# borglab/gtsam

Hardware: NVIDIA H100
Metric: LM iterations/sec (linearize+solve) on BAL-style graph (higher is better)
Workload: dtype f32 Jacobians + f64 solve

## Files before the change

gtsam_b200/csrc/engine.cu:

```cuda
#include <algorithm>
#include <chrono>
#include <climits>
#include <cmath>
#include <cstdlib>
#include <dlfcn.h>
#include <cstring>
#include <limits>
#include <memory>
#include <thread>

#include "kernels.cuh"

namespace b200 {

static thread_local std::string g_err;

template <class F>
static void parallel_chunks(int64_t n, F f) {
  int nt = (int)std::min<int64_t>(std::max(1u, std::thread::hardware_concurrency()), 16);
  if (const char* e = getenv("B200_SETUP_THREADS")) nt = std::min(16, std::max(1, atoi(e)));
  nt = (int)std::min<int64_t>(nt, std::max<int64_t>(1, n / 65536));
  if (nt <= 1) { f((int64_t)0, n, 0); return; }
  std::vector<std::thread> pool;
  for (int t = 0; t < nt; t++) pool.emplace_back([=, &f]() { f(n * t / nt, n * (t + 1) / nt, t); });
// ... 163 lines not shown
  for (auto& g : p->groups) {
    if (!g.count) continue;
    PhaseScope ps(p, g.count >= 4096 ? PH_LINEARIZE : PH_LINEARIZE_MINOR);
    const int nb = (int)((g.count + 127) / 128);
    const bool proj = g.type == B200_FACTOR_PROJECTION_CAL3S2 || g.type == B200_FACTOR_SFM_BUNDLER;
    if (proj && p->lin_variant == 4) {
      if (g.type == B200_FACTOR_PROJECTION_CAL3S2)
        DISPATCH_JT(p, launch_k(linearize_kernel<B200_FACTOR_PROJECTION_CAL3S2, JT, 4>, dim3(nb), dim3(128), 0, st, view(g), ectx(p, p->d_values)));
      else
        DISPATCH_JT(p, launch_k(linearize_kernel<B200_FACTOR_SFM_BUNDLER, JT, 4>, dim3(nb), dim3(128), 0, st, view(g), ectx(p, p->d_values)));
    } else
    DISPATCH_JT(p, DISPATCH_TYPE(g.type, (launch_k(linearize_kernel<TY, JT>, dim3(nb), dim3(128), 0, st, view(g), ectx(p, p->d_values)))));
    p->ctx->launches++;
  }
  B200_CUDA(cudaGetLastError());
  p->linearized = true;
  p->hdiag_valid = false;
  return B200_OK;
}

static int enqueue_hdiag(b200_problem* p) {
  cudaStream_t st = p->ctx->stream;
  B200_CUDA(cudaMemsetAsync(p->d_hdiag, 0, (size_t)p->ndelta * sizeof(double), st));
  for (auto& g : p->groups) {
    if (!g.count) continue;
    const int nb = (int)((g.count + 127) / 128);
    if (g.type == B200_FACTOR_JACOBIAN) launch_k(hdiag_jacobian_kernel, dim3(nb), dim3(128), 0, st, jview(g), (const int*)p->d_var_dof, p->d_hdiag);
    else if (g.type == B200_FACTOR_HESSIAN) launch_k(hdiag_hessian_kernel, dim3(nb), dim3(128), 0, st, jview(g), (const int*)p->d_var_dof, p->d_hdiag);
    else DISPATCH_JT(p, DISPATCH_TYPE(g.type, (launch_k(hdiag_kernel<TY, JT>, dim3(nb), dim3(128), 0, st, view(g), p->d_var_dof, p->d_hdiag))));
    p->ctx->launches++;
  }
  B200_CUDA(cudaGetLastError());
  return allreduce_sum(p, p->d_hdiag, (size_t)p->ndelta);
}

static int enqueue_solve(b200_problem* p, bool damped, int diagonal, double min_diag, double max_diag) {
  cudaStream_t st = p->ctx->stream;
  b200_ctx* ctx = p->ctx;
  const TreeView t = tview(p);
  {
    PhaseScope ps(p, PH_MEMSET);
    if (p->zero_doubles) B200_CUDA(cudaMemsetAsync(p->d_arena, 0, (size_t)p->zero_doubles * sizeof(double), st));
    if (p->df_sync_ints) B200_CUDA(cudaMemsetAsync(p->d_df_sync, 0, (size_t)p->df_sync_ints * sizeof(int), st));
    if (p->topx_doubles && p->d_topx) B200_CUDA(cudaMemsetAsync(p->d_topx, 0, (size_t)p->topx_doubles * sizeof(double), st));
  }
  {
    PhaseScope ps(p, PH_ASSEMBLE);
    for (auto& g : p->groups) {
      if (!g.n_nonleaf) continue;
      const int nb = (int)((g.count + 127) / 128);
      if (g.type == B200_FACTOR_JACOBIAN) launch_k(assemble_jacobian_kernel, dim3(nb), dim3(128), 0, st, jview(g), t);
      else if (g.type == B200_FACTOR_HESSIAN) launch_k(assemble_hessian_kernel, dim3(nb), dim3(128), 0, st, jview(g), t);
      else DISPATCH_JT(p, DISPATCH_TYPE(g.type, (launch_k(assemble_kernel<TY, JT>, dim3(nb), dim3(128), 0, st, view(g), t))));
      ctx->launches++;
    }
  }
  if (damped) {
    PhaseScope ps(p, PH_DAMP);
    if (diagonal && !p->hdiag_valid) { const int rc = enqueue_hdiag(p); if (rc) return rc; p->hdiag_valid = true; }
    launch_k(damp_kernel, dim3((int)((p->ndelta + 255) / 256)), dim3(256), 0, st, p->d_arena, p->d_diag_index, (int)p->ndelta, p->d_lambda,
                                                                diagonal ? p->d_hdiag.get() : nullptr, min_diag, max_diag);
    ctx->launches++;
  }
  if (p->n_fused) {
    PhaseScope ps(p, PH_LEAF);
    GroupTable gt;
    for (size_t gi = 0; gi < p->groups.size(); gi++) gt.g[gi] = view(p->groups[gi]);
    const double* hd = (damped && diagonal) ? p->d_hdiag.get() : nullptr;
    if (p->leaf_run_end[0] > p->leaf_run_begin[0]) {
      const int nr = p->leaf_run_end[0] - p->leaf_run_begin[0], nb = (nr + kWarpsPerBlock - 1) / kWarpsPerBlock;
      const size_t sm = (size_t)kWarpsPerBlock * p->leaf_lb_cap * sizeof(double);
      DISPATCH_JT(p, launch_k(leaf_fused_kernel<JT>, dim3(nb), dim3(kWarpsPerBlock * 32), sm, st, t, gt, p->d_fused_list, p->d_fused_run_ptr + p->leaf_run_begin[0], nr,
                                                           p->d_fused_fac_ptr, p->d_fused_fac, p->d_lambda, hd, min_diag, max_diag,
                                                           p->d_scalars, p->leaf_lb_cap, 0));
      ctx->launches++;
    }
    for (int kd = 1; kd <= 2 && p->schur_mma; kd++) {
      const int nr = p->leaf_run_end[kd] - p->leaf_run_begin[kd];
      if (nr <= 0) continue;
      const int* runs = p->d_fused_run_ptr + p->leaf_run_begin[kd];
      const int dc = kd == 1 ? 6 : 9, maxw = p->leaf_max_w[kd], nt8 = (maxw + 7) / 8;
      const int mmax = std::max(1, (maxw - 1) / dc), sa = (dc < 8 ? 8 : 16) * kSmPA + kSmPadA;
      const size_t jb = p->jac_f32 ? sizeof(float) : sizeof(double);
      const size_t sm = std::max((size_t)4 * (3 + 8 * nt8) * kSmKS * sizeof(double) + (size_t)4 * (2 * mmax * sa + 2 * 6 * 32) * jb,
                                 (size_t)64 * nt8 * nt8 * sizeof(double));
      bool done = false;
#define B200_LAUNCH_FUSED(DC_, T_)                                                                                                    \
      if (!done && dc == DC_ && nt8 <= T_) {                                                                                          \
        DISPATCH_JT(p, launch_k(leaf_point_fused_mma_kernel<DC_, T_, JT>, dim3(nr), dim3(128), sm, st, t, gt, (const int*)p->d_fused_list, runs, \
                 (const double*)p->d_lambda, hd, min_diag, max_diag, p->d_scalars, (const int2*)p->d_pt_tab, (const int64_t*)p->d_pt_off)); \
        done = true;                                                                                                                  \
      }
      B200_LAUNCH_FUSED(6, 4) B200_LAUNCH_FUSED(6, 5) B200_LAUNCH_FUSED(6, 7)
      B200_LAUNCH_FUSED(9, 4) B200_LAUNCH_FUSED(9, 5) B200_LAUNCH_FUSED(9, 7) B200_LAUNCH_FUSED(9, 10)
#undef B200_LAUNCH_FUSED
      if (!done) { set_error("leaf_point_fused_mma_kernel: separator wider than the compiled tile counts"); return B200_CUDA_ERROR; }
      ctx->launches++;
    }
    for (int kd = 1; kd <= 2 && !p->schur_mma; kd++) {
      if (p->leaf_run_end[kd] <= p->leaf_run_begin[kd]) continue;
      const int i0 = p->leaf_pos_begin[kd], i1 = p->leaf_pos_end[kd];
      const int nb = (int)(((int64_t)(i1 - i0) * 8 + 127) / 128);
#define B200_LAUNCH_POINT(DC_)                                                                                                        \
      DISPATCH_JT(p, launch_k(leaf_point_factor_kernel<DC_, JT>, dim3(nb), dim3(128), 0, st, t, gt, (const int*)p->d_fused_list, i0, i1, \
               (const int*)p->d_fused_fac_ptr, (const int2*)p->d_fused_fac, (const double*)p->d_lambda, hd, min_diag, max_diag,        \
               p->d_scalars, (const int2*)p->d_pt_tab, (const int64_t*)p->d_pt_off));
      if (kd == 1) { B200_LAUNCH_POINT(6) } else { B200_LAUNCH_POINT(9) }
#undef B200_LAUNCH_POINT
      ctx->launches++;
    }
  }
  if (p->n_fused && !p->schur_mma) {
    PhaseScope ps(p, PH_LEAF_SCHUR);
    GroupTable gt;
    for (size_t gi = 0; gi < p->groups.size(); gi++) gt.g[gi] = view(p->groups[gi]);
    for (int kd = 1; kd <= 2; kd++) {
      const int nr = p->leaf_run_end[kd] - p->leaf_run_begin[kd];
      if (nr <= 0) continue;
      const int* runs = p->d_fused_run_ptr + p->leaf_run_begin[kd];
      const int ntd = (p->leaf_max_w[kd] + 2) / 3, ntiles = ntd * (ntd + 1) / 2;
      const int thr = ntiles <= 96 ? 96 : 128, tpt = (ntiles + thr - 1) / thr;
#define B200_LAUNCH_SCHUR(DC_, T_, P_)                                                                                               \
      if (kd == (DC_ == 6 ? 1 : 2) && tpt == T_ && p->schur_pb == P_)                                                                \
        DISPATCH_JT(p, launch_k(leaf_point_schur_kernel<DC_, T_, P_, JT>, dim3(nr), dim3(thr), 0, st, t, gt, (const int*)p->d_fused_list, runs, \
                 (const int*)p->d_fused_fac_ptr, (const int2*)p->d_fused_fac));
      if (tpt > (kd == 1 ? 2 : 3)) { set_error("leaf_point_schur_kernel: separator wider than the compiled tile counts"); return B200_CUDA_ERROR; }
      B200_LAUNCH_SCHUR(6, 1, 4) B200_LAUNCH_SCHUR(6, 2, 4)
      B200_LAUNCH_SCHUR(6, 1, 6) B200_LAUNCH_SCHUR(6, 2, 6)
      B200_LAUNCH_SCHUR(9, 1, 4) B200_LAUNCH_SCHUR(9, 2, 4) B200_LAUNCH_SCHUR(9, 3, 4)
      B200_LAUNCH_SCHUR(9, 1, 6) B200_LAUNCH_SCHUR(9, 2, 6) B200_LAUNCH_SCHUR(9, 3, 6)
#undef B200_LAUNCH_SCHUR
      ctx->launches++;
    }
  }
  for (size_t l = 0; l < p->levels.size(); l++) {
    if ((int)l == p->n_sub_levels && ctx->world > 1 && !p->top_staged) {
      PhaseScope ps(p, PH_ALLREDUCE);
      const int rc = allreduce_sum(p, p->d_arena, (size_t)p->top_doubles);
      if (rc) return rc;
    }
    const LevelPlan& L = p->levels[l];
    auto launch_df = [&](int slot, const int4* tasks, int ntasks, bool trace) {
      DfView v;
      v.tasks = tasks; v.ntasks = ntasks;
      v.ctrl = p->d_df_sync + 2 * slot; v.done = p->d_df_sync + p->df_ctrl_ints; v.flags = v.done + p->sym.ncliques;
      v.flag_off = p->d_df_flag_off; v.expect = p->d_df_expect;
      v.trace = trace ? p->d_df_trace.get() : nullptr;
      v.winv = p->d_winv; v.winv_off = p->d_winv_off;
      v.warm_ctas = getenv("B200_DF_NO_WARM") ? 0 : 3 * ctx->sm_count;
      if (p->df_minb == 3) launch_k(front_df_kernel<3>, dim3(ntasks), dim3(kDfThreads), (size_t)kDfSmemBytes, st, t, v, p->d_scalars);
      else launch_k(front_df_kernel<2>, dim3(ntasks), dim3(kDfThreads), (size_t)kDfSmemBytes, st, t, v, p->d_scalars);
      ctx->launches++;
    };
    for (int ph = 0; ph < 2; ph++)
      if ((int)l == p->df_level[ph] && p->df_ntasks[ph] && !(ph == 1 && p->top_staged)) {
        PhaseScope ps(p, PH_ELIM_LARGE);
        launch_df(ph, p->d_df_tasks[ph], p->df_ntasks[ph], ph == 0);
      }
    if (p->top_staged)
      for (size_t s = 0; s < p->ts_level.size(); s++)
        if (p->ts_level[s] == (int)l) {
          {
            PhaseScope ps(p, PH_ALLREDUCE);
            const int rc = reduce_top_stage(p, s);
            if (rc) return rc;
          }
          if (p->ts_task_count[s]) {
            PhaseScope ps(p, PH_ELIM_LARGE);
// ... 639 lines not shown
  int64_t ngroups = 0;
  Packed pk;
  std::vector<char> fused, is_top;
  std::vector<int> clique_owner, factor_owner, top_owner;
  std::vector<int> fused_list, run_ptr;
  std::vector<int> leaf_kind;
  std::vector<std::vector<int2>> hkeys; std::vector<std::vector<int4>> hscat;
};

static int setup_symbolic(b200_problem* p, ProblemPlan& P) {
  if (const int rc = P.d ? pack_and_symbolic(P.d, &P.pk) : pack_linear(P.ld, &P.pk)) return rc;
  const int64_t n = P.d ? P.d->nvars : P.ld->nvars;
  P.ngroups = P.d ? P.d->ngroups : P.ld->ngroups + P.ld->nhgroups;
  p->nvars = n; p->nval = P.pk.val_off[n]; p->ndelta = P.pk.var_dof[n]; p->nfactors = P.pk.total;
  if (P.d) p->var_type.assign(P.d->var_type, P.d->var_type + n);
  p->groups.resize(P.ngroups);
  for (int64_t gi = 0; gi < P.ngroups; gi++) {
    auto& g = p->groups[gi];
    const PackedGroup& q = P.pk.groups[gi];
    g.type = q.type; g.noise_kind = q.noise_kind; g.per_factor = q.per_factor; g.noise_size = q.noise_size;
    g.d = q.d; g.ncols = q.ncols; g.arity = q.arity; g.meas = q.meas; g.count = q.count; g.pos = q.pos;
    g.robust_kind = q.robust_kind; g.robust_param = q.robust_param;
    g.col0[0] = 0;
    for (int a = 0; a < B200_JACOBIAN_MAX_ARITY; a++) g.col0[a + 1] = g.col0[a] + (a < q.arity ? q.dims[a] : 0);
    g.col0[q.arity + 1] = g.col0[q.arity] + 1;
  }
  p->sym = std::move(P.pk.sym);
  return B200_OK;
}
static int setup_values(b200_problem* p, ProblemPlan& P) {
  if (P.d) {
    B200_CUDA(upload(p->d_values, P.d->values, (size_t)p->nval, p->ctx->stream));
    B200_CUDA(p->d_new_values.alloc(p->nval));
    B200_CUDA(upload(p->d_val_off, P.pk.val_off, p->ctx->stream));
    B200_CUDA(upload(p->d_var_type, p->var_type, p->ctx->stream));
    B200_CUDA(upload(p->d_cal, P.d->cal, (size_t)P.d->ncal * 5, p->ctx->stream));
  }
  B200_CUDA(p->d_delta.alloc(p->ndelta));
  B200_CUDA(cudaMemsetAsync(p->d_delta, 0, std::max<int64_t>(1, p->ndelta) * sizeof(double), p->ctx->stream));
  B200_CUDA(p->d_hdiag.alloc(p->ndelta));
  B200_CUDA(upload(p->d_var_dof, P.pk.var_dof, p->ctx->stream));
  return B200_OK;
}
static int setup_leaf_runs(b200_problem* p, ProblemPlan& P) {
  const Symbolic& S = p->sym;
  const b200_ctx* ctx = p->ctx;
  shard_plan(S, P.ngroups, p->nfactors, ctx->world, &P.fused, &P.is_top, &P.clique_owner, &P.factor_owner, P.d != nullptr, &P.top_owner);
  p->top_staged = ctx->world > 1 && getenv("B200_REPLICATED_TOP") == nullptr;
  std::vector<int>& fused_list = P.fused_list;
  for (int64_t c = 0; c < S.ncliques; c++)
    if (P.fused[c] && P.clique_owner[c] == p->ctx->rank) fused_list.push_back((int)c);
  auto sig_cmp = [&](int a, int b) {
    if (S.parent[a] != S.parent[b]) return S.parent[a] < S.parent[b] ? -1 : 1;
    const int64_t la = S.sep_ptr[a + 1] - S.sep_ptr[a], lb = S.sep_ptr[b + 1] - S.sep_ptr[b];
    if (la != lb) return la < lb ? -1 : 1;
    for (int64_t q = 0; q < la; q++) {
      const int64_t va = S.sep_vars[S.sep_ptr[a] + q], vb = S.sep_vars[S.sep_ptr[b] + q];
      if (va != vb) return va < vb ? -1 : 1;
    }
    return 0;
  };
  std::vector<int> cf_count(S.ncliques, 0), cf_mask(S.ncliques, 0);
  std::vector<int>& kind = P.leaf_kind;
  kind.assign(S.ncliques, 0);
  for (int64_t gi = 0; P.d && gi < P.d->ngroups; gi++)
    for (int64_t i = 0; i < P.d->groups[gi].count; i++) {
      const int c = S.fac_clique[p->groups[gi].pos[i]];
      if (P.fused[c]) { cf_count[c]++; cf_mask[c] |= 1 << P.d->groups[gi].type; }
    }
  const bool fast = !getenv("B200_NO_POINT_KERNEL");
  for (int c : fused_list) {
    const int64_t nsep = S.sep_ptr[c + 1] - S.sep_ptr[c];
    const bool point = S.front_ptr[c + 1] - S.front_ptr[c] == 1 && P.d->var_type[S.front_vars[S.front_ptr[c]]] == B200_VAR_POINT3;
    if (!fast || !point || cf_count[c] != nsep || cf_count[c] > kPtMaxObs || cf_count[c] < 1) continue;
    if (cf_mask[c] == (1 << B200_FACTOR_PROJECTION_CAL3S2)) kind[c] = 1;
    else if (cf_mask[c] == (1 << B200_FACTOR_SFM_BUNDLER)) kind[c] = 2;
  }
  std::sort(fused_list.begin(), fused_list.end(), [&](int a, int b) {
    if (kind[a] != kind[b]) return kind[a] < kind[b];
    const int s = sig_cmp(a, b);
    return s != 0 ? s < 0 : a < b;
  });
  const int nfl = (int)fused_list.size();
  int run_max_pt = getenv("B200_NO_LEAF_RUNS") ? 1 : std::max(1, std::min(64, nfl / (ctx->sm_count * 8)));
  if (getenv("B200_LEAF_RUN_MAX")) run_max_pt = std::max(1, atoi(getenv("B200_LEAF_RUN_MAX")));
  std::vector<int>& run_ptr = P.run_ptr;
  run_ptr.push_back(0);
  for (int i = 1; i <= nfl; i++) {
    const int kprev = kind[fused_list[i - 1]];
    const int rmax = kprev == 0 ? 1 : run_max_pt;
    if (i == nfl || i - run_ptr.back() >= rmax || kind[fused_list[i]] != kprev || sig_cmp(fused_list[i - 1], fused_list[i]) != 0)
      run_ptr.push_back(i);
  }
  p->n_runs = (int)run_ptr.size() - 1;
  for (int kd = 0, r = 0; kd < 3; kd++) {
    p->leaf_run_begin[kd] = r;
    while (r < p->n_runs && kind[fused_list[run_ptr[r]]] == kd) r++;
    p->leaf_run_end[kd] = r;
    p->leaf_pos_begin[kd] = run_ptr[p->leaf_run_begin[kd]];
    p->leaf_pos_end[kd] = run_ptr[r];
  }
  for (int c : fused_list) {
    if (kind[c] == 0) p->leaf_lb_cap = std::max(p->leaf_lb_cap, S.nf[c] * (S.nf[c] + S.ns[c] + 1));
    p->leaf_max_w[kind[c]] = std::max(p->leaf_max_w[kind[c]], S.ns[c] + 1);
  }
  p->n_fused = nfl;
  p->schur_pb = (getenv("B200_SCHUR_PB") && atoi(getenv("B200_SCHUR_PB")) == 6) ? 6 : 4;
  p->schur_mma = !(getenv("B200_SCHUR_MMA") && atoi(getenv("B200_SCHUR_MMA")) == 0);
  if (getenv("B200_LIN_VARIANT")) p->lin_variant = atoi(getenv("B200_LIN_VARIANT"));
  return B200_OK;
}
static int setup_offsets(b200_problem* p, ProblemPlan& P) {
  const Symbolic& S = p->sym;
  p->h_off.assign(S.ncliques + 1, 0);
  p->h_ld.assign(S.ncliques, 0);
  int64_t o = 0;
  std::vector<int64_t> order(S.ncliques);
  for (int64_t c = 0; c < S.ncliques; c++) order[c] = c;
  std::stable_sort(order.begin(), order.end(), [&](int64_t a, int64_t b) { return (P.is_top[a] ? S.level[a] : -1) < (P.is_top[b] ? S.level[b] : -1); });
  for (int pass = 0; pass < 2; pass++) {
    for (int64_t oc = 0; oc < S.ncliques; oc++) {
      const int64_t c = pass == 0 ? order[oc] : oc;
      if (!P.fused[c] && (P.is_top[c] != 0) == (pass == 0)) {
        const int64_t nn = S.nf[c] + S.ns[c] + 1; p->h_ld[c] = (int)nn;
        if (pass == 1 && P.clique_owner[c] != p->ctx->rank) { p->h_off[c] = 0; continue; }
        p->h_off[c] = o; o += nn * nn;
      }
    }
    if (pass == 0) p->top_doubles = o;
  }
  p->zero_doubles = o;
  for (int64_t c = 0; c < S.ncliques; c++)
    if (P.fused[c]) {
      const int64_t nn = S.nf[c] + S.ns[c] + 1; p->h_ld[c] = S.nf[c];
      if (P.clique_owner[c] != p->ctx->rank) { p->h_off[c] = 0; continue; }
      p->h_off[c] = o; o += (int64_t)S.nf[c] * nn;
    }
  p->arena_doubles = o;
  p->h_off[S.ncliques] = o;
  return B200_OK;
}
static int setup_linear_groups(b200_problem* p, ProblemPlan& P) {
  if (!P.ld) return B200_OK;
  const Symbolic& S = p->sym;
  const b200_linear_desc* ld = P.ld;
  for (int64_t gi = 0; gi < P.ngroups; gi++) {
    auto& g = p->groups[gi];
    const bool hess = gi >= ld->ngroups;
    const int ar = g.arity;
    g.full_count = g.count;
    for (int64_t i = 0; i < g.full_count; i++) if (P.factor_owner[g.pos[i]] == p->ctx->rank) g.local_index.push_back(i);
    const int64_t count = (int64_t)g.local_index.size();
    g.count = count;
    std::vector<int> jkeys((size_t)count * ar), jslots((size_t)count * ar), jclique((size_t)count);
    for (int64_t li = 0; li < count; li++) {
      const int64_t pos = g.pos[g.local_index[li]];
      jclique[li] = S.fac_clique[pos];
      for (int a = 0; a < ar; a++) {
        jkeys[(size_t)li * ar + a] = (int)P.pk.fkeys[P.pk.fptr[pos] + a];
        jslots[(size_t)li * ar + a] = S.fac_slots[P.pk.fptr[pos] + a];
      }
    }
    g.n_nonleaf = count;
    B200_CUDA(upload(g.d_jkeys, jkeys, p->ctx->stream));
    B200_CUDA(upload(g.d_jslots, jslots, p->ctx->stream));
    B200_CUDA(upload(g.d_jclique, jclique, p->ctx->stream));
    B200_CUDA(g.d_J.alloc((size_t)count * g.d * g.ncols));
    const int rc = hess ? upload_jacobian_group(p, g, ld->hgroups[gi - ld->ngroups].info, nullptr)
                        : upload_jacobian_group(p, g, ld->groups[gi].Ab, ld->groups[gi].sigmas);
    if (rc) return rc;
  }
  return B200_OK;
}
static int setup_typed_groups(b200_problem* p, ProblemPlan& P) {
  if (!P.d) return B200_OK;
  const Symbolic& S = p->sym;
  const std::vector<int>& fused_list = P.fused_list;
  const bool reorder_leaf_factors = getenv("B200_NO_FACTOR_REORDER") == nullptr;
  std::vector<int> leaf_list_pos(S.ncliques, INT_MAX);
  for (size_t i = 0; i < fused_list.size(); i++) if (P.leaf_kind[fused_list[i]] > 0) leaf_list_pos[fused_list[i]] = (int)i;
  P.hkeys.resize(P.ngroups);
  P.hscat.resize(P.ngroups);
  for (int64_t gi = 0; gi < P.ngroups; gi++) {
    const b200_factor_group& s = P.d->groups[gi];
    auto& g = p->groups[gi];
    std::vector<int64_t>& keep = g.local_index;
    for (int64_t i = 0; i < s.count; i++) if (P.factor_owner[g.pos[i]] == p->ctx->rank) keep.push_back(i);
// ... 1339 lines not shown
```

gtsam_b200/csrc/kernels.cuh:

```cuda
#pragma once
#include <climits>

#include "engine.cuh"
#ifdef B200_EMULATE
#include "cuda_emu_full.h"
#define B200_DYN_SMEM(T, name) T* name = (T*)b200_emu::dyn_smem()
#else
#define B200_DYN_SMEM(T, name) extern __shared__ T name[]
#endif
#include "factors.cuh"

namespace b200 {

constexpr int kSmallMaxN = 48;
constexpr int kWarpsPerBlock = 4;
constexpr int kLeafMaxF = 6;
constexpr int kLeafMaxFN = 768;
constexpr int kMaxGroups = 8;

struct GroupTable { GroupView g[kMaxGroups]; };
__constant__ int kFD[B200_NUM_FACTOR_TYPES] = {6, 6, 3, 2, 2, 9, 3, 3};
__constant__ int kFN1[B200_NUM_FACTOR_TYPES] = {6, 6, 3, 6, 9, 9, 3, 3};
__constant__ int kFN2[B200_NUM_FACTOR_TYPES] = {6, 0, 0, 3, 3, 0, 3, 0};
constexpr int kMaxPairs = 96;
// ... 903 lines not shown
      const int i0 = 3 * ti[u], j0 = 3 * tj[u];
      const int ci = i0 / DC, cj = j0 / DC;
      const int oi = i0 - ci * DC, oj = j0 - cj * DC;
      for (int pt = 0; pt < nbp; pt++) {
        const double* Si = sS[buf][pt] + 3 * i0;
        const double* Sj = sS[buf][pt] + 3 * j0;
#pragma unroll
        for (int r = 0; r < 3; r++) {
          double si[3], sj[3];
#pragma unroll
          for (int x = 0; x < 3; x++) { si[x] = Si[3 * x + r]; sj[x] = Sj[3 * x + r]; }
#pragma unroll
          for (int x = 0; x < 3; x++)
#pragma unroll
            for (int y = 0; y < 3; y++) acc[u][x][y] -= si[x] * sj[y];
        }
        if (tj[u] < ts) {
          if (ci == cj) {
            const JT* A = sA[buf][pt][ci];
#pragma unroll
            for (int x = 0; x < 3; x++)
#pragma unroll
              for (int y = 0; y < 3; y++)
                acc[u][x][y] += (double)A[2 * (oi + x)] * (double)A[2 * (oj + y)] + (double)A[2 * (oi + x) + 1] * (double)A[2 * (oj + y) + 1];
          }
        } else if (ti[u] < ts) {
          const JT* A = sA[buf][pt][ci];
#pragma unroll
          for (int x = 0; x < 3; x++) acc[u][x][0] += (double)A[2 * (oi + x)] * (double)A[2 * DC] + (double)A[2 * (oi + x) + 1] * (double)A[2 * DC + 1];
        } else {
          for (int fi = 0; fi < m; fi++) {
            const JT* A = sA[buf][pt][fi];
            acc[u][0][0] += (double)A[2 * DC] * (double)A[2 * DC] + (double)A[2 * DC + 1] * (double)A[2 * DC + 1];
          }
        }
      }
    }
    __syncthreads();
  }
  double* P = t.arena + t.off[p];
  const int pn = t.nf[p] + t.ns[p] + 1;
  const int* map = t.ea_map + t.ea_ptr[c0];
#pragma unroll
  for (int u = 0; u < TPT; u++) {
    if (ti[u] < 0) continue;
#pragma unroll
    for (int x = 0; x < 3; x++)
#pragma unroll
      for (int y = 0; y < 3; y++) {
        const int i = 3 * ti[u] + x, j = 3 * tj[u] + y;
        if (i <= j && j < w) {
          const int a = map[i], bq = map[j];
          const int lo = a < bq ? a : bq, hi = a < bq ? bq : a;
          atomicAdd(P + lo + (size_t)hi * pn, acc[u][x][y]);
        }
      }
  }
}

#ifdef B200_EMULATE
__device__ __forceinline__ void dmma_m8n8k4(double& d0, double& d1, double a, double b) {
  const int lane = threadIdx.x & 31, i = lane >> 2, j0 = 2 * (lane & 3);
  for (int k = 0; k < 4; k++) {
    const double ak = __shfl_sync(0xffffffffu, a, 4 * i + k);
    const double b0 = __shfl_sync(0xffffffffu, b, 4 * j0 + k), b1 = __shfl_sync(0xffffffffu, b, 4 * (j0 + 1) + k);
    d0 += ak * b0;
    d1 += ak * b1;
  }
}
#else
__device__ __forceinline__ void dmma_m8n8k4(double& d0, double& d1, double a, double b) {
  asm volatile("mma.sync.aligned.m8n8k4.row.col.f64.f64.f64.f64 {%0,%1}, {%2}, {%3}, {%0,%1};\n"
               : "+d"(d0), "+d"(d1)
               : "d"(a), "d"(b));
}
#endif

constexpr int kSmMP = 4;
constexpr int kSmKS = 3 * kSmMP;
constexpr int kSmKA = 2 * kSmMP;
constexpr int kSmPA = 12;
constexpr int kSmPadA = 4;

template <int DC, int NTT, typename JT = double>
__global__ void __launch_bounds__(128, (NTT <= 5 && DC == 6) ? 3 : (NTT <= 7 ? 2 : 1))
leaf_point_fused_mma_kernel(TreeView t, GroupTable gt, const int* __restrict__ list, const int* __restrict__ run_ptr,
                            const double* __restrict__ lambda_ptr, const double* __restrict__ hdiag, double min_diag,
                            double max_diag, Scalars* sc, const int2* __restrict__ pt_tab, const int64_t* __restrict__ pt_off) {
  pdl_sync();
  constexpr int MP = kSmMP, KS = kSmKS, PA = kSmPA;
  constexpr int CP = DC < 8 ? 8 : 16, CT = CP / 8;
  constexpr int NAT = CT * (CT + 1) / 2;
  constexpr int SA = CP * PA + kSmPadA;
  constexpr int MC = (8 * NTT - 1) / DC < kPtMaxObs ? (8 * NTT - 1) / DC : kPtMaxObs;
  B200_DYN_SMEM(double, sm_dyn);
  __shared__ int64_t sOff[4][2][MP];
  __shared__ int sC[4][2][MP];
  __shared__ int sSlot[4][2][32];
  const double lambda = *lambda_ptr;
  const int tid = threadIdx.x, lane = tid & 31, warp = tid >> 5, g = lane >> 2, q = lane & 3;
  const int pl = lane >> 3, fl = lane & 7;
  const int r0 = run_ptr[blockIdx.x], r1 = run_ptr[blockIdx.x + 1];
  const int c0 = list[r0];
  const int s = t.ns[c0], w = s + 1;
  const int m = s / DC;
  const int NT = (w + 7) >> 3, WP = 8 * NT;
  const int f_doubles = (3 + WP) * KS;
  const int a_elems = 2 * m * SA;
  double* sF = sm_dyn + (size_t)warp * f_doubles;
  double* sS = sF + 3 * KS;
  JT* sA = reinterpret_cast<JT*>(sm_dyn + (size_t)4 * f_doubles) + (size_t)warp * (a_elems + 2 * 6 * 32);
  JT* sP = sA + a_elems;
  double acc[NTT][NTT][2];
  double accA[MC][NAT][2];
#pragma unroll
  for (int a = 0; a < NTT; a++)
#pragma unroll
    for (int b = 0; b < NTT; b++) acc[a][b][0] = acc[a][b][1] = 0.0;
#pragma unroll
  for (int ci = 0; ci < MC; ci++)
#pragma unroll
    for (int x = 0; x < NAT; x++) accA[ci][x][0] = accA[ci][x][1] = 0.0;
  for (int e = lane; e < f_doubles; e += 32) if (e / KS >= 3 + w) sF[e] = 0.0;
  for (int e = lane; e < a_elems; e += 32) { const int r = e % SA; if (r / PA > DC || r % PA >= kSmKA) sA[e] = (JT)0; }
  const int npts = r1 - r0, nmb = (npts + MP - 1) / MP;
  const JT* srcJ = nullptr;
  int cntJ = 0;
  int slotJ = -1, cJ = 0;
  int64_t offJ = 0;
  auto load_idx = [&](int mb) {
    const int b0 = r0 + MP * mb, nb = min(MP, r1 - b0);
    slotJ = -1;
    if (pl < nb) {
      const int2 rec = pt_tab[(size_t)(b0 + pl) * kPtMaxObs + fl];
      offJ = pt_off[b0 + pl];
      cJ = list[b0 + pl];
      if (rec.x >= 0) {
        const GroupView& gv = gt.g[rec.y >> 8];
        cntJ = (int)gv.count;
        srcJ = reinterpret_cast<const JT*>(gv.J) + rec.x;
        slotJ = rec.y & 0xff;
      }
    }
  };
  auto issue = [&](int buf, int nb) {
    JT* A = sA + buf * m * SA;
    if (slotJ >= 0) {
      JT* dst = A + slotJ * SA + 2 * pl;
#pragma unroll
      for (int cc = 0; cc < DC; cc++) {
        cp_async_el(dst + cc * PA, srcJ + (size_t)(2 * cc) * cntJ);
        cp_async_el(dst + cc * PA + 1, srcJ + (size_t)(2 * cc + 1) * cntJ);
      }
      cp_async_el(dst + DC * PA, srcJ + (size_t)(2 * (DC + 3)) * cntJ);
      cp_async_el(dst + DC * PA + 1, srcJ + (size_t)(2 * (DC + 3) + 1) * cntJ);
      JT* P = sP + buf * 6 * 32 + lane;
#pragma unroll
      for (int el = 0; el < 6; el++) cp_async_el(P + 32 * el, srcJ + (size_t)(2 * DC + el) * cntJ);
    }
    cp_async_commit();
    sSlot[warp][buf][lane] = slotJ;
    if (fl == 0 && pl < nb) { sOff[warp][buf][pl] = offJ; sC[warp][buf][pl] = cJ; }
    if (nb < MP)
      for (int e = lane; e < m * (DC + 1) * (kSmKA - 2 * nb); e += 32) {
        const int cc = e / (kSmKA - 2 * nb);
        A[cc / (DC + 1) * SA + cc % (DC + 1) * PA + 2 * nb + (e - cc * (kSmKA - 2 * nb))] = (JT)0;
      }
  };
  if (warp < nmb) {
    load_idx(warp);
    issue(0, min(MP, npts - MP * warp));
    if (warp + 4 < nmb) load_idx(warp + 4);
  }
  int buf = 0;
  for (int mb = warp; mb < nmb; mb += 4, buf ^= 1) {
    const int nb = min(MP, npts - MP * mb);
    if (mb + 4 < nmb) {
      issue(buf ^ 1, min(MP, npts - MP * (mb + 4)));
      cp_async_wait<1>();
    } else {
      cp_async_wait<0>();
    }
    __syncwarp();
    const JT* A = sA + buf * m * SA;
    {
      const int slot = sSlot[warp][buf][lane];
      const bool live = pl < nb;
      const JT* Al = A + slot * SA + 2 * pl;
      double Ap[2][3], v[9];
#pragma unroll
      for (int i = 0; i < 9; i++) v[i] = 0.0;
      if (slot >= 0) {
        const JT* P = sP + buf * 6 * 32 + lane;
#pragma unroll
        for (int j = 0; j < 3; j++) { Ap[0][j] = (double)P[32 * (2 * j)]; Ap[1][j] = (double)P[32 * (2 * j + 1)]; }
        const double b[2] = {(double)Al[DC * PA], (double)Al[DC * PA + 1]};
        PointFactor::lane_terms(Ap, b, v);
      }
      const int c = live ? sC[warp][buf][pl] : 0;
      const bool hd = hdiag && live;
      PointFactor f;
      f.factor(v, lambda, hd ? hdiag : nullptr, hd ? t.didx + t.didx_ptr[c] : nullptr, min_diag, max_diag);
      if (live) {
        if (fl == 0) {
          if (!f.ok) atomicMax(&sc->fail_code, INT_MAX - c);
          double* F = sF + 3 * pl;
          F[0] = f.r00; F[1] = 0.0; F[2] = 0.0;
          F[KS] = f.r01; F[KS + 1] = f.r11; F[KS + 2] = 0.0;
          F[2 * KS] = f.r02; F[2 * KS + 1] = f.r12; F[2 * KS + 2] = f.r22;
          F[(3 + s) * KS] = f.d0; F[(3 + s) * KS + 1] = f.d1; F[(3 + s) * KS + 2] = f.d2;
        }
        if (slot >= 0) {
          double* F = sS + DC * slot * KS + 3 * pl;
#pragma unroll
          for (int cc = 0; cc < DC; cc++) {
            double s0, s1, s2;
            f.s_col(Ap, (double)Al[cc * PA], (double)Al[cc * PA + 1], s0, s1, s2);
            F[cc * KS] = s0; F[cc * KS + 1] = s1; F[cc * KS + 2] = s2;
          }
        }
      } else {
        for (int col = fl; col < w; col += 8) { double* F = sS + col * KS + 3 * pl; F[0] = F[1] = F[2] = 0.0; }
      }
    }
    __syncwarp();
#pragma unroll 1
    for (int z = 0; z < nb; z++) {
      double* dst = t.arena + sOff[warp][buf][z];
      const double* src = sF + 3 * z;
#pragma unroll 1
      for (int e = lane; e < 3 * (3 + w); e += 32) { const int col = e / 3; dst[e] = src[col * KS + (e - 3 * col)]; }
    }
    if (mb + 8 < nmb) load_idx(mb + 8);
#pragma unroll
    for (int k4 = 0; k4 < KS / 4; k4++) {
      double fr[NTT];
#pragma unroll
      for (int a = 0; a < NTT; a++) fr[a] = a < NT ? sS[(8 * a + g) * KS + 4 * k4 + q] : 0.0;
#pragma unroll
      for (int a = 0; a < NTT; a++)
#pragma unroll
        for (int b = a; b < NTT; b++)
          if (b < NT) dmma_m8n8k4(acc[a][b][0], acc[a][b][1], -fr[a], fr[b]);
    }
#pragma unroll
    for (int ci = 0; ci < MC; ci++) {
      if (ci >= m) break;
#pragma unroll
      for (int k4 = 0; k4 < kSmKA / 4; k4++) {
        double fa[CT];
#pragma unroll
        for (int x = 0; x < CT; x++) fa[x] = (double)A[ci * SA + (8 * x + g) * PA + 4 * k4 + q];
#pragma unroll
        for (int x = 0; x < CT; x++)
#pragma unroll
          for (int y = x; y < CT; y++) dmma_m8n8k4(accA[ci][x * CT - x * (x - 1) / 2 + (y - x)][0], accA[ci][x * CT - x * (x - 1) / 2 + (y - x)][1], fa[x], fa[y]);
      }
    }
    __syncwarp();
  }
  const int p = t.parent[c0];
  if (p < 0) return;
  __syncthreads();
  double* R = sm_dyn;
  for (int round = 0; round < 4; round++) {
    if (warp == round) {
#pragma unroll
      for (int a = 0; a < NTT; a++)
#pragma unroll
        for (int b = a; b < NTT; b++)
          if (b < NT) {
#pragma unroll
            for (int h = 0; h < 2; h++) {
              double* dst = R + (8 * a + g) * WP + 8 * b + 2 * q + h;
              *dst = round == 0 ? acc[a][b][h] : *dst + acc[a][b][h];
            }
          }
      __syncwarp();
#pragma unroll
      for (int ci = 0; ci < MC; ci++) {
        if (ci >= m) break;
#pragma unroll
        for (int x = 0; x < CT; x++)
#pragma unroll
          for (int y = x; y < CT; y++)
#pragma unroll
            for (int h = 0; h < 2; h++) {
              const int lx = 8 * x + g, ly = 8 * y + 2 * q + h;
              if (lx <= ly && ly <= DC) {
                const int i = lx < DC ? ci * DC + lx : s, j = ly < DC ? ci * DC + ly : s;
                R[i * WP + j] += accA[ci][x * CT - x * (x - 1) / 2 + (y - x)][h];
              }
            }
        __syncwarp();
      }
    }
    __syncthreads();
  }
  double* P = t.arena + t.off[p];
  const int pn = t.nf[p] + t.ns[p] + 1;
  const int* map = t.ea_map + t.ea_ptr[c0];
  for (int e = tid; e < w * w; e += 128) {
    const int i = e / w, j = e - i * w;
    if (i > j) continue;
    const int a = map[i], bq = map[j];
    const int lo = a < bq ? a : bq, hi = a < bq ? bq : a;
    atomicAdd(P + lo + (size_t)hi * pn, R[i * WP + j]);
  }
}

}
#include "front_df.cuh"
namespace b200 {

__global__ void __launch_bounds__(kWarpsPerBlock * 32)
backsub_small_kernel(TreeView t, const int* __restrict__ list, int count, double* delta, Scalars* sc) {
  pdl_sync();
  __shared__ double xs[kWarpsPerBlock][kSmallMaxN];
  const int warp = threadIdx.x >> 5, lane = threadIdx.x & 31;
  const int idx = blockIdx.x * kWarpsPerBlock + warp;
  if (idx >= count) return;
  const int c = list[idx];
  const int f = t.nf[c], s = t.ns[c], n = f + s + 1, ld = t.ld[c];
  const double* M = t.arena + t.off[c];
  const int* di = t.didx + t.didx_ptr[c];
  double* x = xs[warp];
  __shared__ double Rst[kWarpsPerBlock][64];
  const bool staged = f <= 8;
  if (staged)
    for (int e = lane; e < f * f; e += 32) Rst[warp][e] = M[(e % f) + (size_t)(e / f) * ld];
  for (int i0 = 0; i0 < f; i0 += 8) {
    double a[8];
#pragma unroll
    for (int k = 0; k < 8; k++) a[k] = 0.0;
    for (int cc = lane; cc < s; cc += 32) {
      const double xsv = delta[di[f + cc]];
      const double* col = M + (size_t)(f + cc) * ld + i0;
#pragma unroll
      for (int k = 0; k < 8; k++)
        if (i0 + k < f) a[k] += col[k] * xsv;
    }
#pragma unroll
    for (int k = 0; k < 8; k++) {
      const double sum = warp_sum(a[k]);
      if (lane == 0 && i0 + k < f) x[i0 + k] = M[(i0 + k) + (size_t)(n - 1) * ld] - sum;
    }
  }
  __syncwarp();
  for (int i = f - 1; i >= 0; i--) {
    if (lane == 0) x[i] = x[i] / (staged ? Rst[warp][i + i * f] : M[i + (size_t)i * ld]);
    __syncwarp();
    const double xi = x[i];
    for (int k = lane; k < i; k += 32) x[k] -= (staged ? Rst[warp][k + i * f] : M[k + (size_t)i * ld]) * xi;
    __syncwarp();
  }
  bool nan = false;
  for (int i = lane; i < f; i += 32) {
    delta[di[i]] = x[i];
    if (isnan(x[i])) nan = true;
  }
  if (nan) atomicMax(&sc->nan_code, INT_MAX - c);
}

constexpr int kBsRows = 64;

template <int DC>
__global__ void __launch_bounds__(128)
backsub_point_kernel(TreeView t, const int* __restrict__ list, int count, double* delta, Scalars* sc) {
  pdl_sync();
  const int sub = threadIdx.x & 7;
  const int idx = (int)((blockIdx.x * blockDim.x + threadIdx.x) >> 3);
  const bool live = idx < count;
  const int c = live ? list[idx] : list[0];
  const int s = t.ns[c];
  const int m = live ? s / DC : 0;
  const double* M = t.arena + t.off[c];
  const int* di = t.didx + t.didx_ptr[c];
  double a0 = 0.0, a1 = 0.0, a2 = 0.0;
  if (sub < m) {
    const double* xs = delta + di[3 + DC * sub];
    const double* S = M + 3 * (3 + DC * sub);
#pragma unroll
    for (int cc = 0; cc < DC; cc++) {
      const double x = xs[cc];
      a0 += S[3 * cc] * x; a1 += S[3 * cc + 1] * x; a2 += S[3 * cc + 2] * x;
    }
  }
#pragma unroll
  for (int o = 4; o > 0; o >>= 1) {
    a0 += __shfl_xor_sync(0xffffffffu, a0, o);
// ... 271 lines not shown
```

Measured before the change: 123.6.

## Size leaf point runs to fill SM waves and parallelize Schur reduction

Run lengths for point-leaf fused MMA blocks are now chosen by binary search, so the total run count fills a few waves of resident blocks, and each signature set is split into balanced runs. The cross-warp reduction of Schur accumulators no longer serializes four rounds with block syncs. Each warp dumps its fragments into its own shared slab, then all threads sum the upper triangle while scattering atomics. The separator map is cached in shared memory. This adds shared memory per block and changes work granularity, which may alter occupancy.

Result: faster. 132.5 (median of 6 runs) (+7.1%).

```diff
diff --git a/gtsam_b200/csrc/engine.cu b/gtsam_b200/csrc/engine.cu
--- a/gtsam_b200/csrc/engine.cu
+++ b/gtsam_b200/csrc/engine.cu
@@ -269,8 +269,9 @@
       const int dc = kd == 1 ? 6 : 9, maxw = p->leaf_max_w[kd], nt8 = (maxw + 7) / 8;
       const int mmax = std::max(1, (maxw - 1) / dc), sa = (dc < 8 ? 8 : 16) * kSmPA + kSmPadA;
       const size_t jb = p->jac_f32 ? sizeof(float) : sizeof(double);
+      const int ct = dc < 8 ? 1 : 2;
       const size_t sm = std::max((size_t)4 * (3 + 8 * nt8) * kSmKS * sizeof(double) + (size_t)4 * (2 * mmax * sa + 2 * 6 * 32) * jb,
-                                 (size_t)64 * nt8 * nt8 * sizeof(double));
+                                 (size_t)4 * 64 * (nt8 * (nt8 + 1) / 2 + mmax * ct * (ct + 1) / 2) * sizeof(double));
       bool done = false;
 #define B200_LAUNCH_FUSED(DC_, T_)                                                                                                    \
       if (!done && dc == DC_ && nt8 <= T_) {                                                                                          \
@@ -1076,15 +1077,43 @@
     return s != 0 ? s < 0 : a < b;
   });
   const int nfl = (int)fused_list.size();
-  int run_max_pt = getenv("B200_NO_LEAF_RUNS") ? 1 : std::max(1, std::min(64, nfl / (ctx->sm_count * 8)));
-  if (getenv("B200_LEAF_RUN_MAX")) run_max_pt = std::max(1, atoi(getenv("B200_LEAF_RUN_MAX")));
+  for (int c : fused_list) {
+    if (kind[c] == 0) p->leaf_lb_cap = std::max(p->leaf_lb_cap, S.nf[c] * (S.nf[c] + S.ns[c] + 1));
+    p->leaf_max_w[kind[c]] = std::max(p->leaf_max_w[kind[c]], S.ns[c] + 1);
+  }
+  constexpr int kLeafRunWaves = 3;
+  std::vector<int> set_ptr(1, 0);
+  for (int i = 1; i <= nfl; i++)
+    if (i == nfl || kind[fused_list[i - 1]] == 0 || kind[fused_list[i]] != kind[fused_list[i - 1]] || sig_cmp(fused_list[i - 1], fused_list[i]) != 0)
+      set_ptr.push_back(i);
+  const char* run_max_env = getenv("B200_LEAF_RUN_MAX");
+  const bool fixed_runs = run_max_env || getenv("B200_NO_LEAF_RUNS");
+  int run_len[3] = {1, 1, 1};
+  for (int kd = 1; kd <= 2; kd++) {
+    std::vector<int> n;
+    for (size_t q = 0; q + 1 < set_ptr.size(); q++) if (kind[fused_list[set_ptr[q]]] == kd) n.push_back(set_ptr[q + 1] - set_ptr[q]);
+    if (n.empty() || getenv("B200_NO_LEAF_RUNS")) continue;
+    if (run_max_env) { run_len[kd] = std::max(1, atoi(run_max_env)); continue; }
+    const int64_t target = (int64_t)kLeafRunWaves * ctx->sm_count * leaf_point_fused_min_blocks(kd == 1 ? 6 : 9, (p->leaf_max_w[kd] + 7) / 8);
+    auto runs = [&](int len) { int64_t r = 0; for (int x : n) r += (x + len - 1) / len; return r; };
+    int lo = std::max(1, std::min(64, nfl / (ctx->sm_count * 8))), hi = *std::max_element(n.begin(), n.end());
+    while (lo < hi) {
+      const int mid = lo + (hi - lo + 1) / 2;
+      if (runs(mid) >= target) lo = mid; else hi = mid - 1;
+    }
+    run_len[kd] = lo;
+  }
   std::vector<int>& run_ptr = P.run_ptr;
   run_ptr.push_back(0);
-  for (int i = 1; i <= nfl; i++) {
-    const int kprev = kind[fused_list[i - 1]];
-    const int rmax = kprev == 0 ? 1 : run_max_pt;
-    if (i == nfl || i - run_ptr.back() >= rmax || kind[fused_list[i]] != kprev || sig_cmp(fused_list[i - 1], fused_list[i]) != 0)
-      run_ptr.push_back(i);
+  for (size_t q = 0; q + 1 < set_ptr.size(); q++) {
+    const int i0 = set_ptr[q], n = set_ptr[q + 1] - i0, len = run_len[kind[fused_list[i0]]];
+    if (fixed_runs) {
+      for (int i = i0 + len; i < i0 + n; i += len) run_ptr.push_back(i);
+      run_ptr.push_back(i0 + n);
+    } else {
+      const int k = (n + len - 1) / len;
+      for (int r = 1; r <= k; r++) run_ptr.push_back(i0 + (int)((int64_t)n * r / k));
+    }
   }
   p->n_runs = (int)run_ptr.size() - 1;
   for (int kd = 0, r = 0; kd < 3; kd++) {
@@ -1093,10 +1122,6 @@
     p->leaf_run_end[kd] = r;
     p->leaf_pos_begin[kd] = run_ptr[p->leaf_run_begin[kd]];
     p->leaf_pos_end[kd] = run_ptr[r];
-  }
-  for (int c : fused_list) {
-    if (kind[c] == 0) p->leaf_lb_cap = std::max(p->leaf_lb_cap, S.nf[c] * (S.nf[c] + S.ns[c] + 1));
-    p->leaf_max_w[kind[c]] = std::max(p->leaf_max_w[kind[c]], S.ns[c] + 1);
   }
   p->n_fused = nfl;
   p->schur_pb = (getenv("B200_SCHUR_PB") && atoi(getenv("B200_SCHUR_PB")) == 6) ? 6 : 4;
diff --git a/gtsam_b200/csrc/kernels.cuh b/gtsam_b200/csrc/kernels.cuh
--- a/gtsam_b200/csrc/kernels.cuh
+++ b/gtsam_b200/csrc/kernels.cuh
@@ -1009,8 +1009,9 @@
 constexpr int kSmPA = 12;
 constexpr int kSmPadA = 4;
 
+constexpr int leaf_point_fused_min_blocks(int dc, int ntt) { return (ntt <= 5 && dc == 6) ? 3 : (ntt <= 7 ? 2 : 1); }
 template <int DC, int NTT, typename JT = double>
-__global__ void __launch_bounds__(128, (NTT <= 5 && DC == 6) ? 3 : (NTT <= 7 ? 2 : 1))
+__global__ void __launch_bounds__(128, leaf_point_fused_min_blocks(DC, NTT))
 leaf_point_fused_mma_kernel(TreeView t, GroupTable gt, const int* __restrict__ list, const int* __restrict__ run_ptr,
                             const double* __restrict__ lambda_ptr, const double* __restrict__ hdiag, double min_diag,
                             double max_diag, Scalars* sc, const int2* __restrict__ pt_tab, const int64_t* __restrict__ pt_off) {
@@ -1032,6 +1033,8 @@
   const int s = t.ns[c0], w = s + 1;
   const int m = s / DC;
   const int NT = (w + 7) >> 3, WP = 8 * NT;
+  __shared__ int sMap[8 * NTT];
+  if (tid < w) { const int pp = t.parent[c0]; if (pp >= 0) sMap[tid] = t.ea_map[t.ea_ptr[c0] + tid]; }
   const int f_doubles = (3 + WP) * KS;
   const int a_elems = 2 * m * SA;
   double* sF = sm_dyn + (size_t)warp * f_doubles;
@@ -1188,51 +1191,50 @@
   }
   const int p = t.parent[c0];
   if (p < 0) return;
+  const int ntp = NT * (NT + 1) / 2, wstride = 64 * (ntp + m * NAT);
   __syncthreads();
-  double* R = sm_dyn;
-  for (int round = 0; round < 4; round++) {
-    if (warp == round) {
-#pragma unroll
-      for (int a = 0; a < NTT; a++)
-#pragma unroll
-        for (int b = a; b < NTT; b++)
-          if (b < NT) {
-#pragma unroll
-            for (int h = 0; h < 2; h++) {
-              double* dst = R + (8 * a + g) * WP + 8 * b + 2 * q + h;
-              *dst = round == 0 ? acc[a][b][h] : *dst + acc[a][b][h];
-            }
-          }
-      __syncwarp();
-#pragma unroll
-      for (int ci = 0; ci < MC; ci++) {
-        if (ci >= m) break;
-#pragma unroll
-        for (int x = 0; x < CT; x++)
-#pragma unroll
-          for (int y = x; y < CT; y++)
-#pragma unroll
-            for (int h = 0; h < 2; h++) {
-              const int lx = 8 * x + g, ly = 8 * y + 2 * q + h;
-              if (lx <= ly && ly <= DC) {
-                const int i = lx < DC ? ci * DC + lx : s, j = ly < DC ? ci * DC + ly : s;
-                R[i * WP + j] += accA[ci][x * CT - x * (x - 1) / 2 + (y - x)][h];
-              }
-            }
-        __syncwarp();
-      }
-    }
-    __syncthreads();
-  }
+  {
+    double* W = sm_dyn + (size_t)warp * wstride + 2 * lane;
+#pragma unroll
+    for (int a = 0; a < NTT; a++)
+#pragma unroll
+      for (int b = a; b < NTT; b++)
+        if (b < NT) {
+          double* dst = W + 64 * (a * NT - a * (a - 1) / 2 + (b - a));
+          dst[0] = acc[a][b][0]; dst[1] = acc[a][b][1];
+        }
+#pragma unroll
+    for (int ci = 0; ci < MC; ci++) {
+      if (ci >= m) break;
+#pragma unroll
+      for (int x = 0; x < NAT; x++) {
+        double* dst = W + 64 * (ntp + ci * NAT + x);
+        dst[0] = accA[ci][x][0]; dst[1] = accA[ci][x][1];
+      }
+    }
+  }
+  __syncthreads();
   double* P = t.arena + t.off[p];
   const int pn = t.nf[p] + t.ns[p] + 1;
-  const int* map = t.ea_map + t.ea_ptr[c0];
-  for (int e = tid; e < w * w; e += 128) {
-    const int i = e / w, j = e - i * w;
-    if (i > j) continue;
-    const int a = map[i], bq = map[j];
+  for (int e = tid; e < w * (w + 1) / 2; e += 128) {
+    int i, j;
+    tri_decode(e, i, j);
+    const int si = (i >> 3) * NT - (i >> 3) * ((i >> 3) - 1) / 2 + ((j >> 3) - (i >> 3));
+    const int so = 64 * si + 8 * (i & 7) + (j & 7);
+    int cf = -1, cl = -1, lx = 0, ly = 0;
+    if (i < s && (j == s || i / DC == j / DC)) { cf = cl = i / DC; lx = i - cf * DC; ly = j == s ? DC : j - cf * DC; }
+    else if (i == s) { cf = 0; cl = m - 1; lx = ly = DC; }
+    const int ao = 64 * (ntp + (lx >> 3) * CT - (lx >> 3) * ((lx >> 3) - 1) / 2 + ((ly >> 3) - (lx >> 3))) + 8 * (lx & 7) + (ly & 7);
+    double v = 0.0;
+#pragma unroll
+    for (int wp = 0; wp < 4; wp++) {
+      const double* W = sm_dyn + (size_t)wp * wstride;
+      v = wp == 0 ? W[so] : v + W[so];
+      for (int ci = cf; ci <= cl && cf >= 0; ci++) v += W[ao + 64 * NAT * ci];
+    }
+    const int a = sMap[i], bq = sMap[j];
     const int lo = a < bq ? a : bq, hi = a < bq ? bq : a;
-    atomicAdd(P + lo + (size_t)hi * pn, R[i * WP + j]);
+    atomicAdd(P + lo + (size_t)hi * pn, v);
   }
 }
 
diff --git a/profiles/point_leaf_stream.py b/profiles/point_leaf_stream.py
--- /dev/null
+++ b/profiles/point_leaf_stream.py
@@ -0,0 +1,148 @@
+#!/usr/bin/env python
+import argparse
+import json
+import os
+import subprocess
+import sys
+import time
+
+import numpy as np
+
+ROOT = os.path.dirname(os.path.dirname(os.path.abspath(__file__)))
+sys.path.insert(0, ROOT)
+
+KERNELS = ("leaf_point_fused_mma_kernel", "backsub_point_kernel", "backsub_large_kernel", "front_df_kernel", "linerr_kernel")
+
+
+def leaf_bytes(prob, jb):
+    from gtsam_b200 import problem as P
+    obs = None
+    dc = 6
+    for g in prob.groups:
+        if g.keys.shape[1] != 2 or P.FACTOR_DIM[g.type] != 2:
+            continue
+        dc = P.factor_ncols(g.type) - 4
+        c = np.bincount(g.keys[:, 1], minlength=prob.nvars)
+        obs = c if obs is None else obs + c
+    m = obs[obs > 0].astype(np.int64)
+    s = dc * m
+    cond = 3 * (s + 4) * 8
+    fused = int(np.sum(m * 2 * (dc + 4) * jb + cond))
+    backsub = int(np.sum(cond + s * 8 + 3 * 8))
+    return fused, backsub, int(m.size)
+
+
+def run_steps(ctx, dev, lm, stream, flush_buf, steps, phases=False):
+    import torch
+    from gtsam_b200 import capi
+    L = dev.L
+    ms = 0.0
+    for it in range(steps):
+        dev.restore_values()
+        capi._check(L.b200_lm_reset(lm.h))
+        with torch.cuda.stream(stream):
+            flush_buf.zero_()
+        a, b = torch.cuda.Event(enable_timing=True), torch.cuda.Event(enable_timing=True)
+        if phases:
+            dev.profile_enable(1 if it == 0 else 2)
+        a.record(stream)
+        lm.iterate()
+        b.record(stream)
+        dev.synchronize()
+        if phases:
+            dev.profile_enable(0)
+        ms += a.elapsed_time(b)
+    return ms / steps, (dev.profile() if phases else None)
+
+
+def open_problem(ctx, prob, jac32):
+    import torch
+    from gtsam_b200 import capi, optimizer
+    dev = capi.DeviceProblem(ctx, prob)
+    if jac32:
+        dev.set_jacobian_precision(True)
+    dev.synchronize()
+    lm = optimizer.LevenbergMarquardtOptimizer(ctx, prob, device_problem=dev)
+    dev.save_values()
+    stream = torch.cuda.ExternalStream(ctx.stream(), device=torch.device("cuda", 0))
+    return dev, lm, stream
+
+
+def main():
+    ap = argparse.ArgumentParser()
+    ap.add_argument("--out", required=True)
+    ap.add_argument("--workloads", default="bal_c5_metis,bal_1m,bal_c3")
+    ap.add_argument("--sweep-workloads", default="bal_c5_metis,bal_1m")
+    ap.add_argument("--sweep", default="32,64,128,256,1024")
+    ap.add_argument("--steps", type=int, default=10)
+    ap.add_argument("--warmup", type=int, default=3)
+    a = ap.parse_args()
+    import torch
+    from torch.profiler import ProfilerActivity, profile
+    from gtsam_b200 import capi, datasets
+
+    os.makedirs(a.out, exist_ok=True)
+    smi = subprocess.run(["nvidia-smi", "--query-gpu=name,power.limit,clocks.max.sm", "--format=csv,noheader"],
+                         capture_output=True, text=True).stdout.strip()
+    print("gpu:", smi, flush=True)
+    ctx = capi.Context(0)
+    flush_buf = torch.empty(256 << 20, dtype=torch.uint8, device="cuda")
+    out = {"gpu": smi, "steps": a.steps, "profile": {}, "sweep": {}}
+    names = list(dict.fromkeys(a.workloads.split(",") + [w for w in a.sweep_workloads.split(",") if w]))
+    for wl in names:
+        t0 = time.perf_counter()
+        prob = datasets.make(wl)
+        jac32 = wl.startswith("bal_c5")
+        jb = 4 if jac32 else 8
+        fused_b, back_b, npts = leaf_bytes(prob, jb)
+        print(f"{wl}: {prob.nfactors} factors, {npts} points, generated in {time.perf_counter() - t0:.1f} s", flush=True)
+        if wl in a.workloads.split(","):
+            os.environ.pop("B200_LEAF_RUN_MAX", None)
+            dev, lm, stream = open_problem(ctx, prob, jac32)
+            run_steps(ctx, dev, lm, stream, flush_buf, a.warmup)
+            with profile(activities=[ProfilerActivity.CUDA]) as prof:
+                run_steps(ctx, dev, lm, stream, flush_buf, a.steps)
+            rec = {"jacobian_bytes": jb, "points": npts, "model_bytes": {"leaf_point_fused_mma_kernel": fused_b,
+                                                                         "backsub_point_kernel": back_b}, "kernels": {}}
+            for ev in prof.key_averages():
+                k = next((k for k in KERNELS if k in ev.key), None)
+                if k is None:
+                    continue
+                us = getattr(ev, "device_time_total", None) or getattr(ev, "cuda_time_total", 0.0)
+                e = rec["kernels"].setdefault(k, {"ms_per_step": 0.0, "launches_per_step": 0.0})
+                e["ms_per_step"] += us * 1e-3 / a.steps
+                e["launches_per_step"] += ev.count / a.steps
+            for k, e in rec["kernels"].items():
+                if k in rec["model_bytes"] and e["launches_per_step"]:
+                    e["gb_per_s"] = rec["model_bytes"][k] / (e["ms_per_step"] / e["launches_per_step"] * 1e-3) / 1e9
+            out["profile"][wl] = rec
+            print(wl, json.dumps({k: {x: round(y, 4) for x, y in e.items()} for k, e in rec["kernels"].items()}), flush=True)
+            del lm
+            dev.close()
+        if wl in a.sweep_workloads.split(","):
+            out["sweep"][wl] = {}
+            for rm in ["auto"] + a.sweep.split(","):
+                if rm == "auto":
+                    os.environ.pop("B200_LEAF_RUN_MAX", None)
+                else:
+                    os.environ["B200_LEAF_RUN_MAX"] = rm
+                dev, lm, stream = open_problem(ctx, prob, jac32)
+                run_steps(ctx, dev, lm, stream, flush_buf, a.warmup)
+                ms, _ = run_steps(ctx, dev, lm, stream, flush_buf, a.steps)
+                _, ph = run_steps(ctx, dev, lm, stream, flush_buf, a.steps, phases=True)
+                r = {"ms_per_step": ms, "leaf_fused": ph["leaf_fused"][0] / a.steps,
+                     "back_substitute": ph["back_substitute"][0] / a.steps}
+                out["sweep"][wl][rm] = r
+                print(wl, "run max", rm, {k: round(v, 4) for k, v in r.items()}, flush=True)
+                del lm
+                dev.close()
+            os.environ.pop("B200_LEAF_RUN_MAX", None)
+        del prob
+    with open(os.path.join(a.out, "point_leaf_stream.json"), "w") as f:
+        json.dump(out, f, indent=1)
+    ctx.close()
+    return 0
+
+
+if __name__ == "__main__":
+    sys.exit(main())
```
